# kokizzu/dragonboat

Measured on AMD Instinct MI355X. Metric: committed entries/sec (node) at 1M active 3-replica groups, 16B payload; %HBM BW, higher is better.
Workload: dtype u64

## Files before the change

dragonboat_amd/csrc/drb_layout.hpp:

```cpp
#pragma once
#include <stdint.h>

#include <hip/hip_runtime.h>

namespace drb {

constexpr uint32_t TAN_LISTS = 64;

__host__ __device__ inline uint64_t lo64(uint4 q) {
  return (uint64_t)q.x | ((uint64_t)q.y << 32);
}
__host__ __device__ inline uint64_t hi64(uint4 q) {
  return (uint64_t)q.z | ((uint64_t)q.w << 32);
}

__host__ __device__ inline uint64_t mix64(uint64_t z) {
  z += 0x9E3779B97F4A7C15ull;
  z = (z ^ (z >> 30)) * 0xBF58476D1CE4E5B9ull;
  z = (z ^ (z >> 27)) * 0x94D049BB133111EBull;
  return z ^ (z >> 31);
}

enum U64Field : int {
  F_TERM = 0,
// ... 72 lines not shown
         : i == PI_PUSHED           ? F_PUSHED_INDEX
                                    : F_PREV_COMMIT;
}
__host__ __device__ inline uint32_t pk_half(const uint32_t *w, int word,
                                            int hi) {
  return (w[word] >> (16 * hi)) & 0xffffu;
}
__host__ __device__ inline void pk_set_half(uint32_t *w, int word, int hi,
                                            uint32_t x) {
  w[word] = (w[word] & ~(0xffffu << (16 * hi))) | ((x & 0xffffu) << (16 * hi));
}
__host__ __device__ inline uint32_t pk_idx_code(uint64_t x, uint64_t base,
                                                bool guard) {
  if (guard && x == ~0ull) return PK_INF16;
  const int64_t d = (int64_t)(x - base);
  if (d < -32767 || d > (guard ? 32766 : 32767)) return PK_ESC16;
  return (uint32_t)(uint16_t)(int16_t)d;
}
__host__ __device__ inline uint64_t pk_idx_value(uint32_t code,
                                                 uint64_t base, bool guard) {
  if (guard && code == PK_INF16) return ~0ull;
  return base + (uint64_t)(int64_t)(int16_t)code;
}
__host__ __device__ inline uint32_t pk_term_code(uint64_t x, uint64_t term) {
  return (x <= term && term - x < PK_ESCU16) ? (uint32_t)(term - x) : PK_ESCU16;
}
__host__ __device__ inline uint32_t pk_u16_code(uint64_t x) {
  return x < PK_ESCU16 ? (uint32_t)x : PK_ESCU16;
}
__host__ __device__ inline uint32_t pk_id_code(uint64_t x) {
  return x < PK_ESC8 ? (uint32_t)x : PK_ESC8;
}

__host__ __device__ inline void pk_encode(uint32_t *w, const uint64_t *vals,
                                          uint64_t *over) {
  const uint64_t last = vals[F_LAST_INDEX], term = vals[F_TERM];
  for (int q = 0; q < 16; ++q) w[q] = 0;
  w[0] = (uint32_t)last;
  w[1] = (uint32_t)(last >> 32);
  w[2] = (uint32_t)term;
  w[3] = (uint32_t)(term >> 32);
  for (int i = 0; i < NUM_PI; ++i) {
    const uint64_t x = vals[pi_field(i)];
    const uint32_t c = pk_idx_code(x, last, i == PI_RING_GUARD);
    if (c == PK_ESC16) over[pi_field(i)] = x;
    pk_set_half(w, 4 + i / 2, i & 1, c);
  }
  const int tf[3] = {F_APPLIED_TO_TERM, F_PREV_TERM, F_SM_TERM};
  const int tw[3] = {11, 11, 12}, th[3] = {0, 1, 0};
  for (int k = 0; k < 3; ++k) {
    const uint32_t c = pk_term_code(vals[tf[k]], term);
    if (c == PK_ESCU16) over[tf[k]] = vals[tf[k]];
    pk_set_half(w, tw[k], th[k], c);
  }
  const int uf[3] = {F_ELECTION_TICK, F_HEARTBEAT_TICK, F_RAND_TIMEOUT};
  const int uw[3] = {12, 13, 13}, uh[3] = {1, 0, 1};
  for (int k = 0; k < 3; ++k) {
    const uint32_t c = pk_u16_code(vals[uf[k]]);
    if (c == PK_ESCU16) over[uf[k]] = vals[uf[k]];
    pk_set_half(w, uw[k], uh[k], c);
  }
  const int df[3] = {F_VOTE, F_LEADER_ID, F_PREV_VOTE};
  for (int k = 0; k < 3; ++k) {
    const uint32_t c = pk_id_code(vals[df[k]]);
    if (c == PK_ESC8) over[df[k]] = vals[df[k]];
    w[14] |= c << (8 * k);
  }
}
__host__ __device__ inline void pk_decode(const uint32_t *w,
                                          const uint64_t *over,
                                          uint64_t *vals) {
  const uint64_t last = (uint64_t)w[0] | ((uint64_t)w[1] << 32);
  const uint64_t term = (uint64_t)w[2] | ((uint64_t)w[3] << 32);
  vals[F_LAST_INDEX] = last;
  vals[F_TERM] = term;
  for (int i = 0; i < NUM_PI; ++i) {
    const uint32_t c = pk_half(w, 4 + i / 2, i & 1);
    vals[pi_field(i)] = c == PK_ESC16
                            ? over[pi_field(i)]
                            : pk_idx_value(c, last, i == PI_RING_GUARD);
  }
  const int tf[3] = {F_APPLIED_TO_TERM, F_PREV_TERM, F_SM_TERM};
  const int tw[3] = {11, 11, 12}, th[3] = {0, 1, 0};
  for (int k = 0; k < 3; ++k) {
    const uint32_t c = pk_half(w, tw[k], th[k]);
    vals[tf[k]] = c == PK_ESCU16 ? over[tf[k]] : term - c;
  }
  const int uf[3] = {F_ELECTION_TICK, F_HEARTBEAT_TICK, F_RAND_TIMEOUT};
  const int uw[3] = {12, 13, 13}, uh[3] = {1, 0, 1};
  for (int k = 0; k < 3; ++k) {
    const uint32_t c = pk_half(w, uw[k], uh[k]);
    vals[uf[k]] = c == PK_ESCU16 ? over[uf[k]] : c;
  }
  const int df[3] = {F_VOTE, F_LEADER_ID, F_PREV_VOTE};
  for (int k = 0; k < 3; ++k) {
    const uint32_t c = (w[14] >> (8 * k)) & 0xffu;
    vals[df[k]] = c == PK_ESC8 ? over[df[k]] : c;
  }
  vals[F_TICK_COUNT] = over[F_TICK_COUNT];
  vals[F_KV_COUNT] = over[F_KV_COUNT];
  for (int f = F_QS_TICK; f <= F_QS_EXIT; ++f) vals[f] = over[f];
  vals[F_RNG] = over[F_RNG];
  vals[F_QS_BASE] = over[F_QS_BASE];
}

enum U32Field : int {
  W_ROLE = 0,
  W_FLAGS,
  W_FB_REASON,
  W_RI_COUNT,
  W_VOTES,
  NUM_U32
};

constexpr uint32_t F_AT_REST = 1u << 16;
constexpr uint32_t F_QUIESCED = 1u << 17;
constexpr uint32_t F_SLOW = 1u << 18;
constexpr uint32_t F_XFER_REQ = 1u << 19;
constexpr int F_XFER_SHIFT = 20;
constexpr uint32_t F_XFER = 0xfu << F_XFER_SHIFT;
constexpr uint32_t F_SAVE_ZERO = 1u << 24;
constexpr uint32_t F_PUBLIC = 0xffffu;

constexpr int MSG_CHUNKS = 2;
constexpr int ENT_META = 3;
constexpr int PROP_META = 3;

__host__ __device__ inline uint32_t prop_fast(uint32_t type, uint64_t client_id,
                                              uint64_t series_id,
                                              uint32_t cmd_len,
                                              uint32_t first_byte,
                                              uint32_t snappy) {
  if (type != 0  && type != 2 ) return 0;
// ... 258 lines not shown
```

dragonboat_amd/csrc/drb_lean.hpp:

```cpp
#pragma once

namespace drb {

#ifndef DRB_LEAN_STRICT
#define DRB_LEAN_STRICT 0
#endif
#ifndef DRB_LEAN_WHY
#define DRB_LEAN_WHY 0
#endif
#ifndef DRB_LEAN_WAVES
#define DRB_LEAN_WAVES 4
#endif
#ifndef DRB_LEAN_FOLLOW_WAVES
#define DRB_LEAN_FOLLOW_WAVES 5
#endif

template <int R, bool LEAD>
__global__ __launch_bounds__(256) __attribute__((amdgpu_waves_per_eu(
    LEAD || R > 3 ? DRB_LEAN_WAVES : DRB_LEAN_FOLLOW_WAVES))) void lean_kernel(
    const View v, RoundParams p) {
  const View *vp = &v;
  const BlockPos bp = block_pos(p);
  const uint32_t slot = (p.slots >> (4 * bp.y)) & 0xfu;
  const uint64_t lrow = (uint64_t)(LEAD ? 0 : 1) * v.R + slot;
  const uint64_t nh = v.act_total[2 * lrow], nl = v.act_total[2 * lrow + 1];
  const uint64_t li = (uint64_t)bp.x * blockDim.x + threadIdx.x;
  if ((uint64_t)bp.x * blockDim.x >= nl) return;
  const uint64_t g = li < nl ? v.act_list[lrow * v.G + nh + li] : v.G;
  __shared__ RemLds<R> rl;
  __shared__ uint32_t oinfo[R * 256];
  Lane L;
  L.rl = &rl;
  L.oi = oinfo;
  L.elo = nullptr;
  L.rq = nullptr;
  L.tid = threadIdx.x;
  L.v = vp;
  L.slot = slot;
  L.g = g;
  L.round = p.round;
  L.rbuf = (uint32_t)((p.round - 1) & 1);
  L.wbuf = (uint32_t)(p.round & 1);
  L.slow = false;
  L.dirty = DRB_REM_DIRTY;
  L.members = false;
  L.peers = false;
  uint32_t c_msgs = 0, c_stepped = 0;
  bool esc = false;
  constexpr int NREC = 1;
  const bool valid = g < v.G;
  const bool qon = v.quiesce;
  uint32_t flags = 0, role = 0, fbw = 0, ric = 0, pcount = 0;
  uint4 pkq[4], meta[R], rec[R][NREC], riq = make_uint4(0, 0, 0, 0);
  uint64_t qsv[5] = {0, 0, 0, 0, 0}, tick_count = 0;
  uint64_t rmatch[R];
  uint32_t rstate[R], ractive[R];
#pragma unroll
  for (int c = 0; c < 4; ++c) pkq[c] = make_uint4(0, 0, 0, 0);
#pragma unroll
  for (int s = 0; s < R; ++s) ractive[s] = 0;
  if (valid) {
    flags = v.u32[u32_ix(v, W_FLAGS, slot, g)];
    role = v.u32[u32_ix(v, W_ROLE, slot, g)];
    fbw = v.u32[u32_ix(v, W_FB_REASON, slot, g)];
    ric = v.u32[u32_ix(v, W_RI_COUNT, slot, g)];
#pragma unroll
    for (int c = 0; c < 4; ++c) pkq[c] = v.pk[pk_ix(v, c, slot, g)];
#pragma unroll
    for (int s = 0; s < R; ++s) {
      if ((uint32_t)s == slot) continue;
      meta[s] = v.mbox_meta[mmeta_ix(v, L.rbuf, s, slot, g)];
#pragma unroll
      for (int j = 0; j < NREC; ++j)
        rec[s][j] = v.mbox[mbox_ix(v, L.rbuf, s, slot,
                                   rec_pos(false, (uint32_t)j, v.MB), 0, g)];
    }
    if (qon) {
      qsv[0] = v.u64[u64_ix(v, F_QS_TICK, slot, g)];
      qsv[1] = v.u64[u64_ix(v, F_QS_IDLE, slot, g)];
      qsv[2] = v.u64[u64_ix(v, F_QS_SINCE, slot, g)];
      qsv[3] = v.u64[u64_ix(v, F_QS_EXIT, slot, g)];
      qsv[4] = v.u64[u64_ix(v, F_QS_BASE, slot, g)];
    }
    if (p.tick) tick_count = v.u64[u64_ix(v, F_TICK_COUNT, slot, g)];
    if (LEAD) {
#pragma unroll
      for (int s = 0; s < R; ++s) {
        if ((uint32_t)s != slot) {
          rmatch[s] = v.rem_match[rem_ix(v, slot, s, g)];
          rstate[s] = v.rem_state[rem_ix(v, slot, s, g)];
        }
        ractive[s] = v.rem_active[rem_ix(v, slot, s, g)];
      }
    }
    if (prop_here(v, p, slot, LEAD))
      pcount = v.prop_count[(uint64_t)p.prop_slot * v.G + g];
    if (ri_here(v, p, slot, LEAD))
      riq = v.ri_in[(uint64_t)p.ri_slot * v.G + g];
  }
  bool active = valid && (flags & DRB_F_HOSTED) &&
                !(flags & (DRB_F_FALLBACK | DRB_F_ERROR)) &&
                ((role == DRB_LEADER) == LEAD);
  if (active) {
    Rep<R> r;
    uint32_t pw0[16];
#pragma unroll
    for (int c = 0; c < 4; ++c) {
      r.pw[4 * c] = pw0[4 * c] = pkq[c].x;
      r.pw[4 * c + 1] = pw0[4 * c + 1] = pkq[c].y;
      r.pw[4 * c + 2] = pw0[4 * c + 2] = pkq[c].z;
      r.pw[4 * c + 3] = pw0[4 * c + 3] = pkq[c].w;
    }
    r.last = (uint64_t)r.pw[0] | ((uint64_t)r.pw[1] << 32);
    r.term = (uint64_t)r.pw[2] | ((uint64_t)r.pw[3] << 32);
    r.base0 = r.last;
    r.leader_id = pd_get(L, r, 1, F_LEADER_ID);
    r.election_tick = pu_get(L, r, 12, 1, F_ELECTION_TICK);
// ... 172 lines not shown
      r.guard_new = ~0ull;
      r.leader_update = false;
      r.oterm = false;
      r.err = false;
      r.qs_new = false;
      r.applied_index = r.sm_index;
      st_f(L, r, F_APPLIED, r.applied_index);
#pragma unroll
      for (int s = 0; s < R; ++s) {
        if ((uint32_t)s == slot) continue;
        if (qon && ((qz_from >> s) & 1)) qs_try_enter(v, r);
        const uint64_t sterm = hi64(meta[s]);
#pragma unroll
        for (int j = 0; j < NREC; ++j) {
          if ((uint32_t)j >= nrec[s]) continue;
          uint64_t plo = 0, phi = 0;
          const Msg m =
              msg_decode(rec[s][j], make_uint4(0, 0, 0, 0), sterm, plo, phi);
          if (qon) qs_record(v, r, m.type);
          if (LEAD)
            leader_heartbeat_resp(L, r, s, m);
          else
            follower_heartbeat(L, r, s, m);
        }
      }
      bool quiet = false;
      if (p.tick && qon) {
        qs_tick_once(v, r);
        quiet = qs_quiesced(r);
      }
      if (p.tick && quiet) {
        r.election_tick++;
      } else if (p.tick) {
        over_st(L, F_TICK_COUNT, tick_count + 1);
        if (LEAD) {
          r.election_tick++;
          if (r.election_tick >= v.election_rtt) {
            r.election_tick = 0;
            if (v.check_quorum) {
#pragma unroll
              for (int s = 0; s < R; ++s) rl.a[s][L.tid] = 0;
              rl.dirty[L.tid] |= 0x88888888u;
            }
          }
          r.heartbeat_tick++;
          if (r.heartbeat_tick >= v.heartbeat_rtt) {
            r.heartbeat_tick = 0;
            broadcast_heartbeat_hint(L, r, 0, 0);
          }
        } else {
          r.election_tick++;
        }
      }
      uint32_t qz_out = 0;
      if (qon && r.qs_new) {
        qz_out = ((1u << R) - 1u) & ~(1u << slot);
        r.nmsgs += R - 1;
      }
      const uint64_t vote = ld_f(L, r, F_VOTE);
      const uint64_t prev_term = ld_f(L, r, F_PREV_TERM);
      const uint64_t prev_vote = ld_f(L, r, F_PREV_VOTE);
      const uint64_t prev_commit = ld_f(L, r, F_PREV_COMMIT);
      const uint64_t confirmed_index = ld_f(L, r, F_CONFIRMED_INDEX);
      const bool state_changed = !(r.term == prev_term && vote == prev_vote &&
                                   r.committed == prev_commit);
      const bool state_empty = r.term == 0 && vote == 0 && r.committed == 0;
      const bool has_update =
// ... 114 lines not shown
```

dragonboat_amd/csrc/drb_recover.hpp:

```cpp
#pragma once
#include <hip/hip_runtime.h>

#include "../../include/drb_engine.h"
#include "drb_layout.hpp"
#include "drb_tanread.hpp"

namespace drb {

struct RecFile {
  uint64_t off, len;
  uint32_t log, pad;
};

struct RecParams {
  uint64_t first_group, n_groups;
  const uint8_t *bytes;
  const RecFile *files;
  const uint32_t *rep_first;
  uint64_t base_index, base_term, seed;
  uint64_t qs_base;
  TrPlan *plans;
  drb_recover_status *st;
};

// ... 131 lines not shown
        mk4(e.client_id, e.series_id);
    uint4 m2 = mk4(e.responded_to, 0);
    m2.z = e.type;
    m2.w = e.cmd_len;
    v.ring[ring_ix(v, L.slot, e.index, 2, L.g)] = m2;
    if (e.term != term_final)
      term_start = e.index + 1;
    else if (term_start > e.index)
      term_start = e.index;
  }

  __device__ bool apply(uint64_t index) {
    const int rc = apply_entry<1, true>(L, r, index);
    if (rc < 0) stop = rc;
    return rc >= 0;
  }
};

__global__ __launch_bounds__(REC_BLOCK) void k_recover_place(View v,
                                                             RecParams p) {
  uint64_t q, g;
  uint32_t slot;
  if (!rec_lane(v, p, &q, &slot, &g)) return;
  const TrPlan pl = p.plans[q];
  if (pl.status != TRS_OK && pl.status != TRS_TAIL_CUT) return;
  const uint32_t f0 = p.rep_first[q];
  const RecFiles files{p.bytes, p.files + f0};
  drb_recover_status &st = p.st[(g - p.first_group) * v.R + slot];
  RingPlacer pc(v, slot, g, p.base_index, p.base_term, pl.term);
  uint64_t applied = p.base_index;
  const bool ok =
      tr_replay(files, pl, rec_limits(v, p, slot, g), pc, &applied);
  st.applied = applied;
  v.u64[u64_ix(v, F_KV_COUNT, slot, g)] += pc.r.kv_added;
  if (!ok) {
    st.status = TRS_APPLY_STOPPED;
    v.u32[u32_ix(v, W_FLAGS, slot, g)] |= DRB_F_FALLBACK;
    v.u32[u32_ix(v, W_FB_REASON, slot, g)] = DRB_FB_RECOVERY;
    return;
  }
  const uint64_t last = pl.last_index, commit = pl.commit;
  const uint64_t high = pl.high_index > last ? pl.high_index : last;
  uint64_t ring_lo = high + 1 > v.W ? high + 1 - v.W : 1;
  if (ring_lo > last) ring_lo = last ? last : 1;
  if (ring_lo <= p.base_index) {
    ring_lo = p.base_index ? p.base_index : 1;
    if (p.base_index) {
      for (uint32_t c = 0; c < v.C16; ++c) pc.chunk(p.base_index, c, 0, 0);
      v.ring[ring_ix(v, slot, p.base_index, 0, g)] = mk4(p.base_term, 0);
      v.ring[ring_ix(v, slot, p.base_index, 1, g)] = mk4(0, 0);
      v.ring[ring_ix(v, slot, p.base_index, 2, g)] = mk4(0, 0);
    }
  }
  uint64_t term_start = pc.term_start < ring_lo ? ring_lo : pc.term_start;
  if (term_start > last + 1) term_start = last + 1;
  uint64_t rng = mix64(p.seed ^ (0xE2ull << 56) ^ (gid(v, slot, g) * v.R + slot));
  rng += 0x9E3779B97F4A7C15ull;
  uint64_t z = rng;
  z = (z ^ (z >> 30)) * 0xBF58476D1CE4E5B9ull;
  z = (z ^ (z >> 27)) * 0x94D049BB133111EBull;
  z ^= z >> 31;
  uint64_t vals[NUM_U64], over[NUM_U64];
  for (int k = 0; k < NUM_U64; ++k) vals[k] = over[k] = 0;
  vals[F_TERM] = pl.term;
  vals[F_VOTE] = pl.vote;
  vals[F_RAND_TIMEOUT] = v.election_rtt + z % v.election_rtt;
  vals[F_COMMITTED] = commit;
// ... 54 lines not shown
```

dragonboat_amd/csrc/drb_step.hpp:

```cpp
#pragma once
#include "../../include/drb_engine.h"
#include "drb_codec.hpp"
#include "drb_layout.hpp"
#include "drb_msg.hpp"
#include "drb_ring.hpp"
#include "drb_snappy.hpp"

namespace drb {

#define DRB_DEV __device__ __forceinline__

#ifndef DRB_LEAD_WAVES
#define DRB_LEAD_WAVES 3
#endif
#ifndef DRB_EXT_LEAD_WAVES
#define DRB_EXT_LEAD_WAVES 3
#endif
#ifndef DRB_SLOW_WAVES
#define DRB_SLOW_WAVES 1
#endif
#ifndef DRB_FOLLOW_WAVES
#define DRB_FOLLOW_WAVES 4
#endif
#ifndef DRB_PROBE_W
// ... 171 lines not shown
    if (r.qs_tick - r.qs_since < 2ull * v.election_rtt) return;
  }
  r.qs_idle = r.qs_tick;
  r.qs_dirty |= 1u;
  if (qs_quiesced(r)) qs_exit(r);
}
template <int R>
DRB_DEV void qs_try_enter(const View &v, Rep<R> &r) {
  if (!qs_quiesced(r) && r.qs_tick - r.qs_exit < 20ull * v.election_rtt)
    return;
  if (!qs_quiesced(r)) qs_enter(r);
}
template <int R>
DRB_DEV bool qs_quiet_tick(const View &v, const Rep<R> &r, uint32_t qz_from) {
  const uint64_t thr = 20ull * v.election_rtt;
  bool q = qs_quiesced(r);
  if (!q && qz_from && !(r.qs_tick - r.qs_exit < thr)) q = true;
  return q || (r.qs_tick + 1 - r.qs_idle > thr);
}
template <int R>
DRB_DEV void qs_tick_once(const View &v, Rep<R> &r) {
  r.qs_tick++;
  if (!qs_quiesced(r) && r.qs_tick - r.qs_idle > 20ull * v.election_rtt)
    qs_enter(r);
}

DRB_DEV uint64_t over_ld(const Lane &L, int f) {
  return L.v->u64[u64_ix(*L.v, f, L.slot, L.g)];
}
DRB_DEV void over_st(const Lane &L, int f, uint64_t x) {
  L.v->u64[u64_ix(*L.v, f, L.slot, L.g)] = x;
}
template <int R>
DRB_DEV uint64_t pi_get(const Lane &L, const Rep<R> &r, int i) {
  const uint32_t c = pk_half(r.pw, 4 + i / 2, i & 1);
  return c == PK_ESC16 ? over_ld(L, pi_field(i))
                       : pk_idx_value(c, r.base0, i == PI_RING_GUARD);
}
template <int R>
DRB_DEV void pi_put(const Lane &L, Rep<R> &r, int i, uint64_t x,
                    uint64_t base) {
  const uint32_t c = pk_idx_code(x, base, i == PI_RING_GUARD);
  if (c == PK_ESC16) over_st(L, pi_field(i), x);
  pk_set_half(r.pw, 4 + i / 2, i & 1, c);
}
template <int R>
DRB_DEV uint64_t pt_get(const Lane &L, const Rep<R> &r, int w, int h, int f) {
  const uint32_t c = pk_half(r.pw, w, h);
  return c == PK_ESCU16 ? over_ld(L, f) : r.term - c;
}
template <int R>
DRB_DEV void pt_put(const Lane &L, Rep<R> &r, int w, int h, int f,
                    uint64_t x) {
  const uint32_t c = pk_term_code(x, r.term);
  if (c == PK_ESCU16) over_st(L, f, x);
  pk_set_half(r.pw, w, h, c);
}
template <int R>
DRB_DEV uint64_t pu_get(const Lane &L, const Rep<R> &r, int w, int h, int f) {
  const uint32_t c = pk_half(r.pw, w, h);
  return c == PK_ESCU16 ? over_ld(L, f) : c;
}
template <int R>
DRB_DEV void pu_put(const Lane &L, Rep<R> &r, int w, int h, int f,
                    uint64_t x) {
  const uint32_t c = pk_u16_code(x);
// ... 1027 lines not shown
      dispatch(L, r, s, m, src);
  } else if (r.role == DRB_FOLLOWER) {
    if (t == DRB_MSG_REQUEST_VOTE)
      el_request_vote(L, r, s, m);
    else if (t == DRB_MSG_READ_INDEX)
      follower_read_index(L, r, m.hint, m.hint_high);
    else if (t == DRB_MSG_LEADER_TRANSFER)
      el_forward_transfer(L, r, m.hint);
    else if (t == DRB_MSG_TIMEOUT_NOW)
      el_timeout_now(L, r);
    else if (t != DRB_MSG_REQUEST_PREVOTE_RESP)
      dispatch(L, r, s, m, src);
  } else {
    if (t == DRB_MSG_REPLICATE || t == DRB_MSG_HEARTBEAT) {
      el_become_follower(L, r, r.term, (uint64_t)s + 1, true);
      dispatch(L, r, s, m, src);
    } else if (t == DRB_MSG_REQUEST_VOTE_RESP) {
      if (r.role == DRB_CANDIDATE) el_candidate_vote_resp(L, r, s, m);
    } else if (t == DRB_MSG_REQUEST_PREVOTE_RESP) {
      if (r.role == DRB_PREVOTE_CANDIDATE) el_pre_vote_resp(L, r, s, m);
    } else if (t == DRB_MSG_REQUEST_VOTE) {
      el_request_vote(L, r, s, m);
    } else if (t == DRB_MSG_READ_INDEX) {
      r.ndropped_ri++;
    } else if (t == DRB_MSG_PROPOSE) {
      r.ndropped_props += m.n;
    }
  }
}

template <int R>
DRB_DEV void el_tick(const Lane &L, Rep<R> &r, bool xfer = false) {
  const View &v = *L.v;
  over_st(L, F_TICK_COUNT, over_ld(L, F_TICK_COUNT) + 1);
  if (r.role == DRB_LEADER) {
    r.election_tick++;
    const bool abort_xfer =
        (r.flags & F_XFER) && r.election_tick >= v.election_rtt;
    if (r.election_tick >= v.election_rtt) {
      r.election_tick = 0;
      if (v.check_quorum) {
        uint32_t c = 0;
#pragma unroll
        for (int s = 0; s < R; ++s) {
          if (is_nonvoting(L, (uint32_t)s)) continue;
          RemoteV x = rem_get<R>(L, s);
          if ((uint32_t)s == L.slot || x.a) c++;
          x.a = 0;
          rem_put<R>(L, s, x);
        }
        if (c < quorum_of<R>(L)) el_become_follower(L, r, r.term, 0, true);
      }
    }
    if (abort_xfer) r.flags &= ~F_XFER;
    r.heartbeat_tick++;
    if (r.heartbeat_tick >= v.heartbeat_rtt) {
      r.heartbeat_tick = 0;
      if (r.role == DRB_LEADER) broadcast_heartbeat(L, r);
    }
    return;
  }
  r.election_tick++;
  if (r.role == DRB_NONVOTING || r.role == DRB_WITNESS) return;
  if (r.election_tick >= ld_f(L, r, F_RAND_TIMEOUT)) {
    r.election_tick = 0;
    el_election(L, r, xfer);
  }
// ... 123 lines not shown
    for (uint32_t t = 0; t < 4; ++t) {
      uint4 *sl = bk + (uint64_t)t * v.KVW;
      const uint4 h = sl[0];
      if (!((h.z >> 31) & 1u)) {
        if (!free_sl) free_sl = sl;
      } else if ((h.z & 0xffu) == klen && lo64(h) == key8) {
        hit = true;
        return sl;
      }
    }
    b = v.kv_ovf_next[b - 1];
  }
  if (!insert || free_sl) return free_sl;
  const unsigned long long nb = atomicAdd(v.kv_ovf_used, 1ull);
  if (nb >= v.kv_ovf_cap) return nullptr;
  v.kv_ovf_next[nb] = *headp;
  *headp = (uint32_t)nb + 1;
  return v.kv_ovf + (uint64_t)nb * 4 * v.KVW;
}

static __device__ __noinline__ uint32_t snappy_to_row(const uint4 *cmd,
                                                      uint4 *row, uint64_t G,
                                                      uint32_t clen,
                                                      uint32_t cap) {
  SnapRowsIn<uint4> in(cmd, G);
  SnapRowsOut<uint4> out(row, G);
  uint32_t n = 0;
  return snappy_decode(in, clen, out, cap, &n) ? 0u : n;
}

template <int R, bool EXT>
DRB_DEV int apply_entry(const Lane &L, Rep<R> &r, uint64_t index) {
  const View &v = *L.v;
  uint4 m0 = v.ring[ring_ix(v, L.slot, index, 0, L.g)];
  uint4 m1 = v.ring[ring_ix(v, L.slot, index, 1, L.g)];
  uint4 m2 = v.ring[ring_ix(v, L.slot, index, 2, L.g)];
  uint64_t term = lo64(m0);
  uint64_t client_id = lo64(m1), series_id = hi64(m1);
  uint32_t type = m2.z, clen = m2.w;
  if (type == DRB_ENTRY_CONFIG_CHANGE) return -1;
  if (client_id == 0) {
    if (clen != 0) return -1;
    r.sm_index = index;
    r.sm_term = term;
    r.applied_any = true;
    return 0;
  }
  if (series_id != 0) return -1;
  Cmd4 cmd;
  cmd.c0 = v.ring[ring_ix(v, L.slot, index, ENT_META, L.g)];
  cmd.c1 = cmd.c2 = cmd.c3 = make_uint4(0, 0, 0, 0);
  if (v.C16 > 1) cmd.c1 = v.ring[ring_ix(v, L.slot, index, ENT_META + 1, L.g)];
  if (v.C16 > 2) cmd.c2 = v.ring[ring_ix(v, L.slot, index, ENT_META + 2, L.g)];
  if (v.C16 > 3) cmd.c3 = v.ring[ring_ix(v, L.slot, index, ENT_META + 3, L.g)];
  uint32_t off = 0, plen = clen;
  const uint4 *pay = nullptr;
  if (type == DRB_ENTRY_ENCODED) {
    if (clen == 0) return -1;
    uint32_t h = cmd_byte(cmd, 0);
    bool snappy = false;
    if constexpr (EXT) snappy = v.snappy && h == 0x02;
    if (snappy) {
      if (clen > v.C16 * 16) return -1;
      uint4 *row = v.snap + snap_ix(v, L.slot, 0, L.g);
      plen = snappy_to_row(v.ring + ring_ix(v, L.slot, index, ENT_META, L.g),
                           row, v.G, clen, v.D16 * 16);
      if (plen == 0) return -1;
      pay = row;
      cmd.c0 = row[0];
      cmd.c1 = cmd.c2 = cmd.c3 = make_uint4(0, 0, 0, 0);
      if (v.D16 > 1) cmd.c1 = row[v.G];
      if (v.D16 > 2) cmd.c2 = row[2 * v.G];
      if (v.D16 > 3) cmd.c3 = row[3 * v.G];
    } else {
      if ((h & 0xf0) != 0 || (h & 0x0e) != 0 || (h & 1)) return -1;
      off = 1;
      plen = clen - 1;
    }
  } else if (type != DRB_ENTRY_APPLICATION) {
    return -1;
  }
  uint64_t key8 = 0;
  uint32_t klen = 0, voff = 0, vlen = 0;
  bool have_k = false, have_v = false;
  uint32_t i = 0;
  while (i < plen) {
    if (off + i + 3 > 64) return -1;
// ... 366 lines not shown
    } else {
      if (LEAD) rq_lo(L, d) = rq_hi(L, d) = 0;
      r.ri_ix[d] = 0;
      r.ri_fr[d] = 0;
      r.ri_cf[d] = 0;
    }
  }
}

template <int R, bool LEAD>
DRB_DEV void store_rep(const Lane &L, Rep<R> &r, uint32_t flags0,
                       uint32_t fb0) {
  const View &v = *L.v;
  const uint64_t base = r.last;
#pragma unroll
  for (int i = PI_APPLIED; i < NUM_PI; ++i) {
    const uint32_t c = pk_half(r.pw, 4 + i / 2, i & 1);
    if (c != PK_ESC16)
      pi_put(L, r, i, pk_idx_value(c, r.base0, false), base);
  }
  pi_put(L, r, PI_COMMITTED, r.committed, base);
  pi_put(L, r, PI_PROCESSED, r.processed, base);
  pi_put(L, r, PI_MARKER, r.marker, base);
  pi_put(L, r, PI_SAVED_TO, r.saved_to, base);
  pi_put(L, r, PI_SM_INDEX, r.sm_index, base);
  pi_put(L, r, PI_APPLIED_INDEX, r.applied_index, base);
  pi_put(L, r, PI_RING_LO, r.ring_lo, base);
  pi_put(L, r, PI_RING_GUARD, r.ring_guard, base);
  pi_put(L, r, PI_TERM_START, r.term_start, base);
  if (r.lid_dirty) pd_put(L, r, 1, F_LEADER_ID, r.leader_id);
  pu_put(L, r, 12, 1, F_ELECTION_TICK, r.election_tick);
  if (LEAD) pu_put(L, r, 13, 0, F_HEARTBEAT_TICK, r.heartbeat_tick);
  if (r.applied_any) pt_put(L, r, 12, 0, F_SM_TERM, r.sm_term);
  if (r.kv_added)
    over_st(L, F_KV_COUNT, over_ld(L, F_KV_COUNT) + r.kv_added);
  r.pw[0] = (uint32_t)r.last;
  r.pw[1] = (uint32_t)(r.last >> 32);
#pragma unroll
  for (int c = 0; c < 4; ++c)
    v.pk[pk_ix(v, c, L.slot, L.g)] =
        make_uint4(r.pw[4 * c], r.pw[4 * c + 1], r.pw[4 * c + 2],
                   r.pw[4 * c + 3]);
  if (r.flags != flags0) v.u32[u32_ix(v, W_FLAGS, L.slot, L.g)] = r.flags;
  if (r.fb != fb0) v.u32[u32_ix(v, W_FB_REASON, L.slot, L.g)] = r.fb;
  if (!LEAD) return;
  v.u32[u32_ix(v, W_RI_COUNT, L.slot, L.g)] = r.ri_count;
  {
    const uint32_t dm = L.dirty ? rl_of<R>(L).dirty[L.tid] : 0xffffffffu;
#pragma unroll
    for (int s = 0; s < R; ++s) {
      const uint32_t d = dm >> (4 * s);
      if (!(d & 15u)) continue;
      RemoteV x = rem_get<R>(L, s);
      if (d & 1u) v.rem_match[rem_ix(v, L.slot, s, L.g)] = x.m;
      if (d & 2u) v.rem_next[rem_ix(v, L.slot, s, L.g)] = x.n;
      if (d & 4u) v.rem_state[rem_ix(v, L.slot, s, L.g)] = x.st;
      if (d & 8u) v.rem_active[rem_ix(v, L.slot, s, L.g)] = x.a;
    }
  }
#pragma unroll
  for (int d = 0; d < DRB_RI_DEPTH; ++d) {
    if ((uint32_t)d >= r.ri_count) continue;
    v.ri_ctx[ri_ix(v, L.slot, d, L.g)] = mk4(rq_lo(L, d), rq_hi(L, d));
    v.ri_idx[ri_ix(v, L.slot, d, L.g)] = mk4(r.ri_ix[d], r.ri_fr[d]);
    v.ri_conf[ri_ix(v, L.slot, d, L.g)] = r.ri_cf[d];
  }
}

// ... 75 lines not shown
      v.prop_count[(uint64_t)p.prop_slot * v.G + g] != 0)
    return false;
  if (ri_here(v, p, slot, lead) &&
      (v.ri_in[(uint64_t)p.ri_slot * v.G + g].x |
       v.ri_in[(uint64_t)p.ri_slot * v.G + g].y))
    return false;
  return true;
}

template <int R, bool LEAD>
DRB_DEV void pre_load(const Lane &L, const RoundParams &p, uint64_t g,
                      Pre<R> &q) {
  const View &v = *L.v;
  const uint32_t slot = L.slot;
  q.flags = v.u32[u32_ix(v, W_FLAGS, slot, g)];
  q.role = v.u32[u32_ix(v, W_ROLE, slot, g)];
  q.fb = v.u32[u32_ix(v, W_FB_REASON, slot, g)];
  q.ri_count = v.u32[u32_ix(v, W_RI_COUNT, slot, g)];
#pragma unroll
  for (int c = 0; c < 4; ++c) q.pk[c] = v.pk[pk_ix(v, c, slot, g)];
#pragma unroll
  for (int s = 0; s < R; ++s) {
    q.meta[s] = make_uint4(0, 0, 0, 0);
    q.maxapp[s] = 0;
    if ((uint32_t)s == slot) continue;
    const bool rm = pair_remote(v, s, slot);
    q.meta[s] =
        (rm ? in_meta(L, s, slot) : v.mbox_meta)[mmeta_ix(v, L.rbuf, s, slot, g)];
    if (!LEAD)
      q.maxapp[s] = (rm ? in_maxapp(L, s, slot)
                        : v.mbox_maxapp)[mmeta_ix(v, L.rbuf, s, slot, g)];
  }
  q.tags = 0;
  if (!p.listed && !v.remote_mask)
    q.tags = v.inbox_tag[((uint64_t)L.rbuf * v.R + slot) * v.G + g];
  q.ri_in = make_uint4(0, 0, 0, 0);
  q.pcount = 0;
  if (ri_here(v, p, slot, LEAD))
    q.ri_in = v.ri_in[(uint64_t)p.ri_slot * v.G + g];
  if (prop_here(v, p, slot, LEAD))
    q.pcount = v.prop_count[(uint64_t)p.prop_slot * v.G + g];
  if (LEAD) {
#pragma unroll
    for (int s = 0; s < R; ++s) {
      q.rem_m[s] = v.rem_match[rem_ix(v, slot, s, g)];
      q.rem_n[s] = v.rem_next[rem_ix(v, slot, s, g)];
      q.rem_st[s] = v.rem_state[rem_ix(v, slot, s, g)];
      q.rem_a[s] = v.rem_active[rem_ix(v, slot, s, g)];
    }
    q.rq_c = v.ri_ctx[ri_ix(v, slot, 0, g)];
    q.rq_i = v.ri_idx[ri_ix(v, slot, 0, g)];
    q.rq_cf = v.ri_conf[ri_ix(v, slot, 0, g)];
  }
}

struct BlockPos {
  uint32_t x, y, gx;
};
DRB_DEV BlockPos block_pos(const RoundParams &p) {
  const uint32_t n = p.nrows ? p.nrows : 1u;
  const uint32_t b = blockIdx.x, gx = gridDim.x / n;
  BlockPos bp;
  bp.gx = p.gx_all ? p.gx_all : gx;
  bp.y = b / gx;
  bp.x = p.blk0 + b % gx;
  return bp;
}
// ... 628 lines not shown
                                 : mb[mbox_ix(v, L.rbuf, s, slot, k, 0, g)];
            uint4 c1 = make_uint4(0, 0, 0, 0);
            if (c0.x & MF_HAS_C1) c1 = mb[mbox_ix(v, L.rbuf, s, slot, k, 1, g)];
            const uint64_t rt =
                (SLOW && (c0.x & MF_TERM_OTHER))
                    ? (rm ? in_rterm(L, s, slot) : v.rterm)[rterm_ix(v, L.rbuf, s, slot,
                                                           k, g)]
                    : sterm;
            const Msg m = msg_decode(c0, c1, rt, prev_lo, prev_hi);
            if (qon)
              qs_record(v, r,
                        (m.type == DRB_MSG_HEARTBEAT ||
                         m.type == DRB_MSG_HEARTBEAT_RESP) && m.hint > 0
                            ? (uint32_t)DRB_MSG_READ_INDEX
                            : m.type);
            if (SLOW)
              el_dispatch(L, r, s, m, src);
            else
              dispatch<R, FWD>(L, r, s, m, src);
          }
        }
      }
      DRB_PH(2);
      bool quiet = false;
      if (p.tick && qon) {
        qs_tick_once(v, r);
        quiet = qs_quiesced(r);
      }
      if (p.tick && quiet) {
        r.election_tick++;
      } else if (SLOW && p.tick) {
        el_tick(L, r);
      } else if (p.tick) {
        over_st(L, F_TICK_COUNT, over_ld(L, F_TICK_COUNT) + 1);
        if (is_leader) {
          r.election_tick++;
          if (r.election_tick >= v.election_rtt) {
            r.election_tick = 0;
            if (v.check_quorum) {
#pragma unroll
              for (int s = 0; s < R; ++s)
                if (!is_nonvoting(L, (uint32_t)s)) rl_of<R>(L).a[s][L.tid] = 0;
              if (L.dirty)
                rl_of<R>(L).dirty[L.tid] |=
                    0x88888888u & ~nv_bits8(nv_mask_of(L));
            }
          }
          r.heartbeat_tick++;
          if (r.heartbeat_tick >= v.heartbeat_rtt) {
            r.heartbeat_tick = 0;
            broadcast_heartbeat(L, r);
          }
        } else {
          r.election_tick++;
        }
      }
      if (nprops && (SLOW ? r.role == DRB_LEADER : LEAD)) {
        if (SLOW && (r.flags & F_XFER))
          r.ndropped_props += nprops;
        else {
          append_props(L, r, p.prop_slot, nprops);
          broadcast_replicate(L, r);
        }
      } else if (FWD && nprops &&
                 (r.role == DRB_FOLLOWER || r.role == DRB_NONVOTING) &&
                 v.fwd_props) {
        forward_props(L, r, p.prop_slot, nprops);
// ... 77 lines not shown
          else
            encode_saves(L, r, save_lo, r.last, crc_tab, c_saved,
                         c_saved_bytes);
        }
        if (has_save) r.saved_to = r.last;
        if (has_apply) r.processed = apply_hi;
        uint64_t la = r.applied_index;
        if (la > 0) {
          if (la > r.committed || la > r.processed)
            set_error(r, DRB_ERR_COMMIT);
          if (la >= r.marker && r.last >= r.marker && la <= r.last) {
            st_f(L, r, F_APPLIED_TO_INDEX, la);
            st_f(L, r, F_APPLIED_TO_TERM, log_term(L, r, la));
            r.marker = la + 1;
          }
        }
      }
      DRB_PH(4);
      if (apply_hi >= apply_lo && apply_lo != 0) {
        uint64_t from = umax64(apply_lo, r.sm_index + 1);
        for (uint64_t idx = from; idx <= apply_hi; ++idx) {
          const int rc = apply_entry<R, EXT>(L, r, idx);
          if (rc < 0) {
            r.flags |= DRB_F_FALLBACK | DRB_F_APPLY_STOPPED;
            r.fb = rc == -2 ? DRB_FB_CAPACITY : DRB_FB_ENTRY_TYPE;
            c_fb = 1;
            break;
          }
          c_applied++;
          if (rc == 1 && (SLOW ? r.role == DRB_LEADER : is_leader))
            c_commit++;
        }
      }
      DRB_PH(5);
      if (LEAD && v.remote_mask) {
        const uint32_t chunks = ENT_META + v.C16;
#pragma unroll
        for (int s = 0; s < R; ++s) {
          if ((uint32_t)s == slot || !pair_remote(v, slot, s)) continue;
          const uint64_t lo = elo_lds[LEAD ? s : 0][threadIdx.x];
          if (lo == ~0ull) continue;
          if (r.last + 1 - lo > v.E || lo < r.ring_lo) {
            set_error(r, DRB_FB_CAPACITY);
            elo_lds[LEAD ? s : 0][threadIdx.x] = ~0ull;
            continue;
          }
          for (uint64_t idx = lo; idx <= r.last; ++idx)
            for (uint32_t c = 0; c < chunks; ++c)
              v.embox[embox_ix(v, L.wbuf, slot, s, (uint32_t)(idx - lo), c,
                               g)] = v.ring[ring_ix(v, slot, idx, c, g)];
          v.elo[mmeta_ix(v, L.wbuf, slot, s, g)] = lo;
        }
        last_final = r.last;
      }
      if (LEAD && p.n_reads)
        serve_reads_lane<EXT>(v, slot, g, r.nrtr, r.sm_index, p.n_reads,
                              p.key_space, c_served, c_deferred);
      sent_c1 = r.c1mask;
      r.ring_guard = r.guard_new;
      if (r.err) {
        r.flags |= DRB_F_ERROR;
        c_err = 1;
      }
      const bool rest = r.sm_index == r.applied_index &&
                        r.committed == r.processed && r.guard_new == ~0ull &&
                        r.nrtr == 0 && !has_save &&
// ... 131 lines not shown
```

Before: 985.4 million.

## Pack tick and KV counters into packed-state word and trim ring loads

Adds 16-bit tick and KV-count accumulators in the otherwise unused word 15 of the packed per-replica state. They fold into the 64-bit overflow fields only when a counter overflows, which removes a u64 load and store per tick and per apply. apply_entry now takes the term from r.term for entries at or after term_start instead of reading chunk 0, and loads command chunks early in the non-extended path. The inbox_tag load is also skipped on non-quiesce tick rounds. Recovery and decode paths fold the packed counters back in, which adds complexity and some risk of inconsistency, for example if other readers of F_KV_COUNT do not fold.

```diff
diff --git a/dragonboat_amd/csrc/drb_layout.hpp b/dragonboat_amd/csrc/drb_layout.hpp
--- a/dragonboat_amd/csrc/drb_layout.hpp
+++ b/dragonboat_amd/csrc/drb_layout.hpp
@@ -128,6 +128,18 @@
   return x < PK_ESC8 ? (uint32_t)x : PK_ESC8;
 }
 
+constexpr int PK_CNT_WORD = 15, PK_CNT_TICK = 0, PK_CNT_KV = 1;
+__host__ __device__ inline uint32_t pk_count_add(uint32_t *w, int hi,
+                                                 uint32_t n) {
+  const uint32_t d = pk_half(w, PK_CNT_WORD, hi) + n;
+  if (d <= 0xffffu) {
+    pk_set_half(w, PK_CNT_WORD, hi, d);
+    return 0;
+  }
+  pk_set_half(w, PK_CNT_WORD, hi, 0);
+  return d;
+}
+
 __host__ __device__ inline void pk_encode(uint32_t *w, const uint64_t *vals,
                                           uint64_t *over) {
   const uint64_t last = vals[F_LAST_INDEX], term = vals[F_TERM];
@@ -193,8 +205,9 @@
     const uint32_t c = (w[14] >> (8 * k)) & 0xffu;
     vals[df[k]] = c == PK_ESC8 ? over[df[k]] : c;
   }
-  vals[F_TICK_COUNT] = over[F_TICK_COUNT];
-  vals[F_KV_COUNT] = over[F_KV_COUNT];
+  vals[F_TICK_COUNT] =
+      over[F_TICK_COUNT] + pk_half(w, PK_CNT_WORD, PK_CNT_TICK);
+  vals[F_KV_COUNT] = over[F_KV_COUNT] + pk_half(w, PK_CNT_WORD, PK_CNT_KV);
   for (int f = F_QS_TICK; f <= F_QS_EXIT; ++f) vals[f] = over[f];
   vals[F_RNG] = over[F_RNG];
   vals[F_QS_BASE] = over[F_QS_BASE];
diff --git a/dragonboat_amd/csrc/drb_lean.hpp b/dragonboat_amd/csrc/drb_lean.hpp
--- a/dragonboat_amd/csrc/drb_lean.hpp
+++ b/dragonboat_amd/csrc/drb_lean.hpp
@@ -52,7 +52,7 @@
   const bool qon = v.quiesce;
   uint32_t flags = 0, role = 0, fbw = 0, ric = 0, pcount = 0;
   uint4 pkq[4], meta[R], rec[R][NREC], riq = make_uint4(0, 0, 0, 0);
-  uint64_t qsv[5] = {0, 0, 0, 0, 0}, tick_count = 0;
+  uint64_t qsv[5] = {0, 0, 0, 0, 0};
   uint64_t rmatch[R];
   uint32_t rstate[R], ractive[R];
 #pragma unroll
@@ -82,7 +82,6 @@
       qsv[3] = v.u64[u64_ix(v, F_QS_EXIT, slot, g)];
       qsv[4] = v.u64[u64_ix(v, F_QS_BASE, slot, g)];
     }
-    if (p.tick) tick_count = v.u64[u64_ix(v, F_TICK_COUNT, slot, g)];
     if (LEAD) {
 #pragma unroll
       for (int s = 0; s < R; ++s) {
@@ -321,7 +320,7 @@
       if (p.tick && quiet) {
         r.election_tick++;
       } else if (p.tick) {
-        over_st(L, F_TICK_COUNT, tick_count + 1);
+        count_add(L, r, PK_CNT_TICK, F_TICK_COUNT, 1);
         if (LEAD) {
           r.election_tick++;
           if (r.election_tick >= v.election_rtt) {
diff --git a/dragonboat_amd/csrc/drb_recover.hpp b/dragonboat_amd/csrc/drb_recover.hpp
--- a/dragonboat_amd/csrc/drb_recover.hpp
+++ b/dragonboat_amd/csrc/drb_recover.hpp
@@ -187,7 +187,12 @@
   const bool ok =
       tr_replay(files, pl, rec_limits(v, p, slot, g), pc, &applied);
   st.applied = applied;
-  v.u64[u64_ix(v, F_KV_COUNT, slot, g)] += pc.r.kv_added;
+  {
+    uint4 c3 = v.pk[pk_ix(v, 3, slot, g)];
+    v.u64[u64_ix(v, F_KV_COUNT, slot, g)] += pc.r.kv_added + (c3.w >> 16);
+    c3.w &= 0xffffu;
+    v.pk[pk_ix(v, 3, slot, g)] = c3;
+  }
   if (!ok) {
     st.status = TRS_APPLY_STOPPED;
     v.u32[u32_ix(v, W_FLAGS, slot, g)] |= DRB_F_FALLBACK;
diff --git a/dragonboat_amd/csrc/drb_step.hpp b/dragonboat_amd/csrc/drb_step.hpp
--- a/dragonboat_amd/csrc/drb_step.hpp
+++ b/dragonboat_amd/csrc/drb_step.hpp
@@ -227,6 +227,11 @@
   L.v->u64[u64_ix(*L.v, f, L.slot, L.g)] = x;
 }
 template <int R>
+DRB_DEV void count_add(const Lane &L, Rep<R> &r, int hi, int f, uint32_t n) {
+  const uint32_t fold = pk_count_add(r.pw, hi, n);
+  if (fold) over_st(L, f, over_ld(L, f) + fold);
+}
+template <int R>
 DRB_DEV uint64_t pi_get(const Lane &L, const Rep<R> &r, int i) {
   const uint32_t c = pk_half(r.pw, 4 + i / 2, i & 1);
   return c == PK_ESC16 ? over_ld(L, pi_field(i))
@@ -1320,7 +1325,7 @@
 template <int R>
 DRB_DEV void el_tick(const Lane &L, Rep<R> &r, bool xfer = false) {
   const View &v = *L.v;
-  over_st(L, F_TICK_COUNT, over_ld(L, F_TICK_COUNT) + 1);
+  count_add(L, r, PK_CNT_TICK, F_TICK_COUNT, 1);
   if (r.role == DRB_LEADER) {
     r.election_tick++;
     const bool abort_xfer =
@@ -1510,10 +1515,19 @@
 template <int R, bool EXT>
 DRB_DEV int apply_entry(const Lane &L, Rep<R> &r, uint64_t index) {
   const View &v = *L.v;
-  uint4 m0 = v.ring[ring_ix(v, L.slot, index, 0, L.g)];
   uint4 m1 = v.ring[ring_ix(v, L.slot, index, 1, L.g)];
   uint4 m2 = v.ring[ring_ix(v, L.slot, index, 2, L.g)];
-  uint64_t term = lo64(m0);
+  Cmd4 cmd;
+  cmd.c1 = cmd.c2 = cmd.c3 = make_uint4(0, 0, 0, 0);
+  if (!EXT) {
+    cmd.c0 = v.ring[ring_ix(v, L.slot, index, ENT_META, L.g)];
+    if (v.C16 > 1) cmd.c1 = v.ring[ring_ix(v, L.slot, index, ENT_META + 1, L.g)];
+    if (v.C16 > 2) cmd.c2 = v.ring[ring_ix(v, L.slot, index, ENT_META + 2, L.g)];
+    if (v.C16 > 3) cmd.c3 = v.ring[ring_ix(v, L.slot, index, ENT_META + 3, L.g)];
+  }
+  uint64_t term = r.term;
+  if (EXT || index < r.term_start)
+    term = lo64(v.ring[ring_ix(v, L.slot, index, 0, L.g)]);
   uint64_t client_id = lo64(m1), series_id = hi64(m1);
   uint32_t type = m2.z, clen = m2.w;
   if (type == DRB_ENTRY_CONFIG_CHANGE) return -1;
@@ -1525,12 +1539,12 @@
     return 0;
   }
   if (series_id != 0) return -1;
-  Cmd4 cmd;
-  cmd.c0 = v.ring[ring_ix(v, L.slot, index, ENT_META, L.g)];
-  cmd.c1 = cmd.c2 = cmd.c3 = make_uint4(0, 0, 0, 0);
-  if (v.C16 > 1) cmd.c1 = v.ring[ring_ix(v, L.slot, index, ENT_META + 1, L.g)];
-  if (v.C16 > 2) cmd.c2 = v.ring[ring_ix(v, L.slot, index, ENT_META + 2, L.g)];
-  if (v.C16 > 3) cmd.c3 = v.ring[ring_ix(v, L.slot, index, ENT_META + 3, L.g)];
+  if (EXT) {
+    cmd.c0 = v.ring[ring_ix(v, L.slot, index, ENT_META, L.g)];
+    if (v.C16 > 1) cmd.c1 = v.ring[ring_ix(v, L.slot, index, ENT_META + 1, L.g)];
+    if (v.C16 > 2) cmd.c2 = v.ring[ring_ix(v, L.slot, index, ENT_META + 2, L.g)];
+    if (v.C16 > 3) cmd.c3 = v.ring[ring_ix(v, L.slot, index, ENT_META + 3, L.g)];
+  }
   uint32_t off = 0, plen = clen;
   const uint4 *pay = nullptr;
   if (type == DRB_ENTRY_ENCODED) {
@@ -1963,8 +1977,6 @@
   pu_put(L, r, 12, 1, F_ELECTION_TICK, r.election_tick);
   if (LEAD) pu_put(L, r, 13, 0, F_HEARTBEAT_TICK, r.heartbeat_tick);
   if (r.applied_any) pt_put(L, r, 12, 0, F_SM_TERM, r.sm_term);
-  if (r.kv_added)
-    over_st(L, F_KV_COUNT, over_ld(L, F_KV_COUNT) + r.kv_added);
   r.pw[0] = (uint32_t)r.last;
   r.pw[1] = (uint32_t)(r.last >> 32);
 #pragma unroll
@@ -2106,7 +2118,7 @@
                         : v.mbox_maxapp)[mmeta_ix(v, L.rbuf, s, slot, g)];
   }
   q.tags = 0;
-  if (!p.listed && !v.remote_mask)
+  if (!p.listed && !v.remote_mask && !(p.tick && !v.quiesce))
     q.tags = v.inbox_tag[((uint64_t)L.rbuf * v.R + slot) * v.G + g];
   q.ri_in = make_uint4(0, 0, 0, 0);
   q.pcount = 0;
@@ -2801,7 +2813,7 @@
       } else if (SLOW && p.tick) {
         el_tick(L, r);
       } else if (p.tick) {
-        over_st(L, F_TICK_COUNT, over_ld(L, F_TICK_COUNT) + 1);
+        count_add(L, r, PK_CNT_TICK, F_TICK_COUNT, 1);
         if (is_leader) {
           r.election_tick++;
           if (r.election_tick >= v.election_rtt) {
@@ -2945,6 +2957,7 @@
             c_commit++;
         }
       }
+      if (r.kv_added) count_add(L, r, PK_CNT_KV, F_KV_COUNT, r.kv_added);
       DRB_PH(5);
       if (LEAD && v.remote_mask) {
         const uint32_t chunks = ENT_META + v.C16;
```

After: 1.031 billion, median of 6. 4.6% higher.
